# voxel-tracer/ag-pathtracer

Measured on AMD Instinct MI355X. Metric: Mrays/sec (primary+secondary) at 1080p/64spp, higher is better.
Workload: dtype f32; 1 GPU; BASELINE configs[2]: Sponza-class closed atrium, 258672 tris / 37 primitives / 35 Disney materials, 1920x1080, 64 spp, PathTracer MaxDepth=5, NEE+MIS; triangles=258672, spp=64

## Files before the change

### ag-pathtracer_amd/csrc/agpt_api.hip

```cpp
#include <hip/hip_runtime.h>

#include <algorithm>
#include <cstdlib>
#include <cstring>
#include <memory>
#include <string>
#include <vector>

#include "agpt_adaptive.h"
#include "agpt_denoise.h"
#include "agpt_internal.h"
#include "agpt_kernels.h"

namespace agpt {

static thread_local std::string g_error;

int fail(int code, const std::string& msg) {
    g_error = msg;
    return code;
}

int interleave_rows(int H, int block, int world, int rank) {
    int rows = 0;
    for (int k = rank, y = k * block; y < H; k += world, y = k * block) rows += std::min(block, H - y);
    return rows;
}

}
using agpt::fail;

static int trace_grid(const agpt_ctx* c) { return c->num_cus * c->blocks_per_cu; }
static int fast_grid(const agpt_ctx* c) { return c->num_cus * c->fast_blocks_per_cu; }

static bool use_fast_trace(const agpt_ctx* c, const DevScene& sc, int count) {
    return count != 1 && sc.n_prims <= 64 * AGPT_MAX_CHUNKS && !c->force_generic;
}

#define AGPT_SMALL_BATCH (48ull << 20)

struct TraceLaunch {
    hipStream_t stream;
    const uint32_t* queue;
    const uint32_t* count_ptr;
    uint32_t count_imm;
    uint32_t* work_head;
    float4 *ro, *rd;
    DevHit* hits;
    uint32_t* occ;
    int count;
    bool small_batch;
    bool recast;
};

template <int MODE, bool COUNT, bool SPILL, bool PEEK>
static void launch_trace_fast(agpt_ctx* c, const DevScene& sc, const TraceLaunch& t) {
    const dim3 block(AGPT_BLOCK), g(fast_grid(c));
    const int refill = MODE == 0 ? c->refill : c->refill_any;
    if (sc.n_prims <= 64) {
        hipLaunchKernelGGL((k_trace_fast<MODE, AGPT_FAST_STACK, false, COUNT, SPILL, PEEK>), g, block, 0, t.stream, sc, t.queue, t.count_ptr,
                           t.count_imm, t.work_head, t.ro, t.rd, t.hits, t.occ, c->counters.p,
                           refill, 0u, c->spill.p, (const unsigned long long*)nullptr, (const uint32_t*)nullptr, MODE == 0 && t.recast,
                           (const float4*)c->beta4.p, c->L4.p);
        return;
    }
    const uint32_t stride = (uint32_t)c->pool_paths;
    if (c->cand_chunks.n < c->pool_paths || c->cand_mask.n < (size_t)((sc.n_prims + 63) / 64) * c->pool_paths) {
        c->note(hipErrorOutOfMemory);
        return;
    }
    hipLaunchKernelGGL((k_candidates<MODE>), dim3(c->num_cus * 8), block, 0, t.stream, sc, t.queue, t.count_ptr, t.count_imm, t.ro, t.rd,
                       c->cand_mask.p, c->cand_chunks.p, stride);
    hipLaunchKernelGGL((k_trace_fast<MODE, AGPT_FAST_STACK, true, COUNT, SPILL, PEEK>), g, block, 0, t.stream, sc, t.queue, t.count_ptr,
                       t.count_imm, t.work_head, t.ro, t.rd, t.hits, t.occ, c->counters.p, refill, stride, c->spill.p,
                       (const unsigned long long*)c->cand_mask.p, (const uint32_t*)c->cand_chunks.p, false, (const float4*)nullptr,
                       (float4*)nullptr);
}

template <bool ANY, bool COUNT, int DEPTH>
static void launch_trace_generic(agpt_ctx* c, int grid, const DevScene& sc, const TraceLaunch& t) {
    hipLaunchKernelGGL((k_trace<ANY, COUNT, DEPTH>), dim3(grid), dim3(AGPT_BLOCK), 0, t.stream, sc, t.queue, t.count_ptr, t.count_imm,
                       t.work_head, t.ro, t.rd, t.hits, t.occ, c->counters.p);
}

template <int MODE>
static void launch_trace(agpt_ctx* c, const DevScene& sc, const TraceLaunch& t) {
    constexpr bool ANY = MODE == 1;
    if (use_fast_trace(c, sc, t.count)) {
        const bool spill = sc.max_depth > AGPT_FAST_STACK;
        if (spill) {
            const size_t need = (size_t)(sc.max_depth - AGPT_FAST_STACK) * (size_t)fast_grid(c) * AGPT_BLOCK;
// ... 159 lines not shown
    if ((rc = c->work.ensure(4096))) return rc;
    if ((rc = c->counters.ensure(1))) return rc;
    c->pool_paths = paths;
    return AGPT_OK;
}

static int fit_pool(agpt_ctx* c, const agpt_scene* s, size_t unit, uint64_t& count) {
    if (unit * (size_t)count > c->pool_paths) {
        size_t free_b = 0, total_b = 0;
        if (hipMemGetInfo(&free_b, &total_b) == hipSuccess) {
            const size_t per_path = AGPT_BYTES_PER_PATH + candidate_bytes_per_path(s->dev.n_prims);
            const size_t avail = free_b + c->pool_paths * per_path;
            const size_t fit = (size_t)((double)avail * 0.9) / per_path;
            while (count > 1 && unit * (size_t)count > fit) count = (count + 1) / 2;
        }
    }
    int rc = ensure_pool(c, unit * (size_t)count, s->dev.n_prims);
    while (rc == AGPT_ERR_NOMEM && count > 1) {
        release_pool(c);
        count = (count + 1) / 2;
        rc = ensure_pool(c, unit * (size_t)count, s->dev.n_prims);
    }
    return rc;
}

static bool shade_tables_fit_lds(const DevScene& d) {
    return agpt::shade_tables_fit_lds(d.n_prims, d.n_materials, d.n_lights) && !getenv("AGPT_SHADE_GLOBAL_TABLES");
}

struct WavefrontRun {
    PathBuffers pb;
    Queues q[2];
    bool mis_mode, timing;
    int count;
    agpt::ShadeVariant shade;
    uint64_t iterations = 0, launches = 0;
};

static int begin_wavefront(agpt_ctx* c, const agpt_scene* s, int enable_counters, bool timing, WavefrontRun& run) {
#define X(T, name) run.pb.name = c->name.p;
    AGPT_POOL_BUFFERS(X)
#undef X
    for (int i = 0; i < 2; i++) {
        Queues& q = run.q[i];
        q.ext = c->q[i][0].p; q.mis = c->q[i][1].p; q.shadow = c->q[i][2].p;
        q.counts = c->qcounts.p + AGPT_NQUEUES * AGPT_QSTRIDE * i;
    }
    run.count = enable_counters == 2 ? 2 : (enable_counters != 0 ? 1 : 0);
    run.mis_mode = use_fast_trace(c, s->dev, run.count) && !c->mis_closest;
    run.timing = timing;
    run.shade.fast = s->shading_arith == AGPT_SHADING_FAST;
    run.shade.level = s->shade_level;
    run.shade.lds_tables = shade_tables_fit_lds(s->dev);
    run.shade.env = !s->envs.empty();
    c->tev_used = 0;
    c->tev_kind.clear();
    HIP_TRY(hipMemsetAsync(c->counters.p, 0, sizeof(DevCounters), c->stream));
    HIP_TRY(hipEventRecord(c->ev[0], c->stream));
    return AGPT_OK;
}

static void set_wavefront_consts(RenderConsts& rc, const WavefrontRun& run, int max_depth, bool trace_all_rays) {
    rc.max_depth = max_depth;
    rc.mis_mode = run.mis_mode ? 1 : 0;
    rc.answer_rays = (run.mis_mode && !trace_all_rays) ? 1 : 0;
}

static int run_wavefront(agpt_ctx* c, agpt_scene* s, const RenderConsts& rcn, WavefrontRun& run) {
    const int count = run.count;
    const PathBuffers& pb = run.pb;
    Queues* const q = run.q;
    const int shade_grid = c->num_cus * c->shade_blocks_per_cu;
    const bool small_batch = (unsigned long long)rcn.NP * (unsigned long long)rcn.S < AGPT_SMALL_BATCH;
    const bool recast = !getenv("AGPT_NO_RECAST");
    const bool side = (c->multi_stream == 2 || (c->multi_stream == 1 && small_batch)) && use_fast_trace(c, s->dev, count) &&
                      s->dev.max_depth <= AGPT_FAST_STACK && s->dev.n_prims <= 64;
    const hipStream_t main_stream = c->stream, mis_stream = side ? c->aux_stream[0] : main_stream,
                      shadow_stream = side ? c->aux_stream[1] : main_stream;
    int cur = 0;
    const int planned = rcn.max_depth + 2;
    for (int it = 0;; it++) {
        if (it >= planned) {
            uint32_t* slot = c->host_pinned + (it & 1) * (AGPT_NQUEUES * AGPT_QSTRIDE);
            HIP_TRY(hipMemcpyAsync(slot, q[cur].counts, ((AGPT_NQUEUES - 1) * AGPT_QSTRIDE + 1) * sizeof(uint32_t), hipMemcpyDeviceToHost, main_stream));
            HIP_TRY(hipEventRecord(c->ev[2 + (it & 1)], main_stream));
            if (it > planned) {
                const uint32_t* seen = c->host_pinned + ((it - 1) & 1) * (AGPT_NQUEUES * AGPT_QSTRIDE);
                HIP_TRY(hipEventSynchronize(c->ev[2 + ((it - 1) & 1)]));
                if (seen[0] == 0 && seen[AGPT_QSTRIDE] == 0 && seen[2 * AGPT_QSTRIDE] == 0) break;
            }
            if (it > 4096) return fail(AGPT_ERR_LIMIT, "agpt: path did not terminate");
        }
        const int nxt = cur ^ 1;
        HIP_TRY(hipMemsetAsync(q[nxt].counts, 0, AGPT_NQUEUES * AGPT_QSTRIDE * sizeof(uint32_t), main_stream));
        HIP_TRY(hipMemsetAsync(c->work.p, 0, 4 * AGPT_FRONTIERS * AGPT_QSTRIDE * sizeof(uint32_t), main_stream));
        uint32_t* const heads[4] = {c->work.p, c->work.p + AGPT_FRONTIERS * AGPT_QSTRIDE, c->work.p + 2 * AGPT_FRONTIERS * AGPT_QSTRIDE,
                                    c->work.p + 3 * AGPT_FRONTIERS * AGPT_QSTRIDE};
        const TraceLaunch ext{main_stream, q[cur].ext, &QCOUNT(q[cur], 0), 0, heads[0], pb.ext_o, pb.ext_d, pb.hit, nullptr,
                              count, small_batch, recast};
        const TraceLaunch mis{mis_stream, q[cur].mis, &QCOUNT(q[cur], 1), 0, heads[1], pb.mis_o, pb.mis_d,
                              run.mis_mode ? nullptr : pb.mis_hit, run.mis_mode ? pb.mis_ok : nullptr, count, small_batch, false};
        const TraceLaunch shadow{shadow_stream, q[cur].shadow, &QCOUNT(q[cur], 2), 0, heads[2], pb.sh_o, pb.sh_d, nullptr, pb.occluded,
                                 count, small_batch, false};
        auto trace_ext = [&]() { launch_trace_timed<0>(c, run.timing, 0, s->dev, ext); };
        auto trace_mis = [&]() {
            if (run.mis_mode) launch_trace_timed<2>(c, run.timing, 1, s->dev, mis);
            else launch_trace_timed<0>(c, run.timing, 1, s->dev, mis);
        };
        auto trace_shadow = [&]() { launch_trace_timed<1>(c, run.timing, 2, s->dev, shadow); };
        if (side) {
            HIP_TRY(hipEventRecord(c->aux_ev[0], main_stream));
            HIP_TRY(hipStreamWaitEvent(mis_stream, c->aux_ev[0], 0));
            HIP_TRY(hipStreamWaitEvent(shadow_stream, c->aux_ev[0], 0));
            trace_mis();
            HIP_TRY(hipEventRecord(c->aux_ev[1], mis_stream));
            trace_shadow();
            HIP_TRY(hipEventRecord(c->aux_ev[2], shadow_stream));
            trace_ext();
            HIP_TRY(hipStreamWaitEvent(main_stream, c->aux_ev[1], 0));
            HIP_TRY(hipStreamWaitEvent(main_stream, c->aux_ev[2], 0));
        } else {
            trace_ext();
            trace_mis();
            trace_shadow();
        }
        agpt::launch_shading(main_stream, run.shade, shade_grid, s->dev, rcn, pb, q[cur], q[nxt], c->counters.p, heads[3]);
        cur = nxt;
        run.iterations++;
        run.launches += 3;
    }
    return AGPT_OK;
}

static void read_counters(const DevCounters& d, agpt_stats* st) {
    st->closest_rays = d.closest_rays;
    st->anyhit_rays = d.anyhit_rays;
// ... 1 lines not shown
    st->root_tests = d.roots;
    st->tri_tests = d.tris;
    st->shaded_vertices = d.shaded;
    st->outliers = d.outliers;
    st->samples = d.samples;
    st->answered_rays = d.answered;
}

static int end_wavefront(agpt_ctx* c) {
    HIP_TRY(hipEventRecord(c->ev[1], c->stream));
    HIP_TRY(hipGetLastError());
    HIP_TRY(c->take_deferred());
    return AGPT_OK;
}

static int fill_stats(agpt_ctx* c, const WavefrontRun& run, uint64_t samples, agpt_stats* stats) {
    if (!stats) return AGPT_OK;
    HIP_TRY(hipStreamSynchronize(c->stream));
    std::memset(stats, 0, sizeof(*stats));
    DevCounters dc;
    HIP_TRY(hipMemcpy(&dc, c->counters.p, sizeof(dc), hipMemcpyDeviceToHost));
    read_counters(dc, stats);
#ifdef AGPT_SHADE_CLOCK
    {
        const double tot = (double)dc.dbg[55];
        static const char* names[8] = {"record loads", "resolve pending", "surface", "emission/termination", "BSDF set-up + light sampling",
                                       "evaluations + ray stores", "final stores", "queue appends + barriers"};
        std::fprintf(stderr, "[shade clock] wave-cycles %.4g:", tot);
        for (int k = 0; k < 8; ++k) std::fprintf(stderr, "  %s %.1f%%", names[k], 100. * dc.dbg[56 + k] / tot);
        std::fprintf(stderr, "\n");
    }
#endif
#ifdef AGPT_TRACE_STATS
    for (int mode = 0; mode < 3; ++mode) {
        const unsigned long long* d = dc.dbg + 16 * mode;
        const double steps = (double)(d[0] + d[1] + d[2]);
        if (steps == 0) continue;
        std::fprintf(stderr,
                     "[trace stats mode %d] steps A/B/C %.3g/%.3g/%.3g (%.1f%%/%.1f%%/%.1f%%)  lanes per step A %.1f B %.1f C %.1f  "
                     "active lanes per step %.1f  refills %.3g (%.1f lanes each)  prefilter batches %.3g\n", mode,
                     (double)d[0], (double)d[1], (double)d[2], 100 * d[0] / steps, 100 * d[1] / steps, 100 * d[2] / steps,
                     d[0] ? (double)d[3] / d[0] : 0., d[1] ? (double)d[4] / d[1] : 0., d[2] ? (double)d[5] / d[2] : 0.,
                     (double)d[6] / steps, (double)d[7], d[7] ? (double)d[8] / d[7] : 0., (double)d[9]);
#ifndef AGPT_TRACE_CLOCK
        std::fprintf(stderr, "[trace stats mode %d] stack pushes %.3g: to depth > 4 %.2f%%  > 6 %.3f%%  > 8 %.4f%%  > 12 %.5f%%\n", mode, (double)d[10],
                     d[10] ? 100. * d[11] / d[10] : 0., d[10] ? 100. * d[12] / d[10] : 0., d[10] ? 100. * d[13] / d[10] : 0.,
                     d[10] ? 100. * d[14] / d[10] : 0.);
#endif
#ifdef AGPT_TRACE_CLOCK
        const double tot = (double)dc.dbg[48 + mode];
        std::fprintf(stderr,
                     "[trace clock mode %d] wave-cycles %.4g: refill %.1f%%  vote %.1f%%  B %.1f%% (of which load wait %.1f%%)  C %.1f%%  A %.1f%%;"
                     "  cycles per step: B %.0f (wait %.0f)  C %.0f  A %.0f  vote %.0f; per refill %.0f\n", mode, tot,
                     100 * d[10] / tot, 100 * d[11] / tot, 100 * d[13] / tot, 100 * d[12] / tot, 100 * d[14] / tot, 100 * d[15] / tot,
                     d[1] ? (double)d[13] / d[1] : 0., d[1] ? (double)d[12] / d[1] : 0., d[2] ? (double)d[14] / d[2] : 0.,
                     d[0] ? (double)d[15] / d[0] : 0., (double)d[11] / steps, d[7] ? (double)d[10] / d[7] : 0.);
#endif
    }
#endif
    stats->samples = samples;
    stats->iterations = run.iterations;
    stats->trace_launches = run.launches;
    float ms = 0;
    HIP_TRY(hipEventElapsedTime(&ms, c->ev[0], c->ev[1]));
    stats->total_ms = ms;
    if (run.timing) {
        for (size_t i = 0; i + 1 < c->tev_used; i += 2) {
            float t = 0;
            HIP_TRY(hipEventElapsedTime(&t, c->tev[i], c->tev[i + 1]));
            const int kind = c->tev_kind[i / 2];
// ... 11 lines not shown
    return AGPT_OK;
}
static int check_tile(const char* fn, const agpt_render_params* rp) {
    if (rp->width <= 0 || rp->height <= 0 || rp->w <= 0 || rp->h <= 0 || rp->x0 < 0 || rp->y0 < 0 || rp->x0 + rp->w > rp->width ||
        rp->y0 + rp->h > rp->height || rp->accum_pitch < rp->x0 + rp->w)
        return fail(AGPT_ERR_INVALID, std::string(fn) + ": bad tile / film");
    return AGPT_OK;
}

static int tile_rows(const char* fn, const agpt_render_params* rp, uint32_t& rows) {
    rows = (uint32_t)rp->h;
    if (rp->interleave_block <= 0) return AGPT_OK;
    if (rp->interleave_world < 1 || rp->interleave_rank < 0 || rp->interleave_rank >= rp->interleave_world || rp->x0 != 0 ||
        rp->y0 != 0 || rp->w != rp->width || rp->h != rp->height)
        return fail(AGPT_ERR_INVALID, std::string(fn) + ": row interleave needs the whole film as tile and 0 <= rank < world");
    rows = (uint32_t)agpt::interleave_rows(rp->height, rp->interleave_block, rp->interleave_world, rp->interleave_rank);
    return AGPT_OK;
}

static RenderConsts tile_consts(const agpt_render_params* rp, uint32_t NP) {
    RenderConsts rc{};
    rc.W = rp->width; rc.H = rp->height; rc.x0 = rp->x0; rc.y0 = rp->y0; rc.w = rp->w; rc.h = rp->h;
    rc.accum_pitch = rp->accum_pitch; rc.accum_row0 = rp->accum_row0; rc.NP = NP;
    rc.il_block = rp->interleave_block; rc.il_world = rp->interleave_world; rc.il_rank = rp->interleave_rank;
    return rc;
}

static uint64_t samples_per_batch(const agpt_render_params* rp, uint32_t NP) {
    return rp->samples_per_batch > 0 ? (uint64_t)rp->samples_per_batch : std::max<uint64_t>(1, (128ull << 20) / NP);
}

static void trace_rays(agpt_ctx* c, const DevScene& sc, uint32_t n, bool any_hit, int count) {
    const TraceLaunch t{c->stream, nullptr, nullptr, n, c->work.p, c->ext_o.p, c->ext_d.p, c->hit.p, c->occluded.p,
                        count, (unsigned long long)n < AGPT_SMALL_BATCH, false};
    if (any_hit) launch_trace<1>(c, sc, t);
    else launch_trace<0>(c, sc, t);
}

int agpt_intersect_device(agpt_scene* s, const agpt_ray* d_rays, int n, agpt_hit* d_out, int any_hit, agpt_stats* stats) {
    if (!s || !d_rays || !d_out || n < 0) return fail(AGPT_ERR_INVALID, "agpt_intersect_device: bad argument");
    if (!s->committed) return fail(AGPT_ERR_INVALID, "agpt_intersect_device: scene not committed");
    if (n == 0) return AGPT_OK;
    agpt_ctx* c = s->ctx;
    HIP_TRY(hipSetDevice(c->device));
    int rc = ensure_pool(c, (size_t)n, s->dev.n_prims);
    if (rc) return rc;
    HIP_TRY(hipMemsetAsync(c->counters.p, 0, sizeof(DevCounters), c->stream));
    HIP_TRY(hipMemsetAsync(c->work.p, 0, AGPT_FRONTIERS * AGPT_QSTRIDE * sizeof(uint32_t), c->stream));
    const dim3 blocks = agpt_blocks((uint64_t)n);
    hipLaunchKernelGGL(k_prepare_rays, blocks, dim3(AGPT_BLOCK), 0, c->stream, d_rays, n, c->ext_o.p, c->ext_d.p);
    HIP_TRY(hipEventRecord(c->ev[0], c->stream));
    const int instrumented = (stats != nullptr && !getenv("AGPT_INTERSECT_TIMING")) ? 1 : 0;
    trace_rays(c, s->dev, (uint32_t)n, any_hit != 0, instrumented);
    HIP_TRY(hipEventRecord(c->ev[1], c->stream));
    hipLaunchKernelGGL(k_export_hits, blocks, dim3(AGPT_BLOCK), 0, c->stream, s->dev, c->hit.p, c->occluded.p, n, any_hit,
                       d_out);
    HIP_TRY(hipStreamSynchronize(c->stream));
    HIP_TRY(hipGetLastError());
    HIP_TRY(c->take_deferred());
    WavefrontRun one{};
    one.launches = 1;
    if ((rc = fill_stats(c, one, 0, stats))) return rc;
    if (stats) stats->trace_ms = stats->total_ms;
    return AGPT_OK;
}

int agpt_intersect_batch(agpt_scene* s, const agpt_ray* rays, int n, agpt_hit* out, int any_hit, agpt_stats* stats) {
// ... 6 lines not shown
    DevBuf<agpt_hit> d_out;
    if (d_rays.alloc((size_t)n) != hipSuccess || d_out.alloc((size_t)n) != hipSuccess)
        return fail(AGPT_ERR_NOMEM, "agpt_intersect_batch: out of device memory");
    HIP_TRY(hipMemcpyAsync(d_rays.p, rays, (size_t)n * sizeof(agpt_ray), hipMemcpyHostToDevice, c->stream));
    int rc = agpt_intersect_device(s, d_rays.p, n, d_out.p, any_hit, stats);
    if (rc) return rc;
    HIP_TRY(hipMemcpy(out, d_out.p, (size_t)n * sizeof(agpt_hit), hipMemcpyDeviceToHost));
    return AGPT_OK;
}

int agpt_render(agpt_scene* s, const agpt_render_params* rp, float* accum_dev, agpt_stats* stats) {
    if (!s || !rp || !accum_dev) return fail(AGPT_ERR_INVALID, "agpt_render: NULL argument");
    if (!s->committed || !s->has_camera) return fail(AGPT_ERR_INVALID, "agpt_render: scene not committed or camera not set");
    int rc;
    if ((rc = check_tile("agpt_render", rp)) || (rc = check_depth("agpt_render", rp->max_depth))) return rc;
    if (rp->spp_count < 0) return fail(AGPT_ERR_INVALID, "agpt_render: bad sample range");
    agpt_ctx* c = s->ctx;
    HIP_TRY(hipSetDevice(c->device));
    uint32_t rows;
    if ((rc = tile_rows("agpt_render", rp, rows))) return rc;
    if (rows == 0) return AGPT_OK;
    const uint32_t NP = (uint32_t)rp->w * rows;
    uint64_t batch = std::min<uint64_t>(samples_per_batch(rp, NP), (uint64_t)std::max(1, rp->spp_count));
    if ((uint64_t)NP * batch > 0x7FFFFFFFull) return fail(AGPT_ERR_LIMIT, "agpt_render: batch too large");
    if ((rc = fit_pool(c, s, NP, batch))) return rc;
    const int S = (int)batch;
    s->dev.cam = s->cam;

    WavefrontRun run;
    if ((rc = begin_wavefront(c, s, rp->enable_counters, rp->enable_timing != 0 && stats != nullptr, run))) return rc;
    RenderConsts rcn = tile_consts(rp, NP);
    rcn.seed_base = rp->seed_base;
    set_wavefront_consts(rcn, run, rp->max_depth, rp->trace_all_rays != 0);
    for (int s0 = rp->spp_begin; s0 < rp->spp_begin + rp->spp_count; s0 += S) {
        rcn.s0 = s0;
        rcn.S = std::min(S, rp->spp_begin + rp->spp_count - s0);
        const uint32_t total = NP * (uint32_t)rcn.S;
        hipLaunchKernelGGL(k_generate, agpt_blocks(total), dim3(AGPT_BLOCK), 0, c->stream, s->dev, rcn, run.pb,
                           run.q[0]);
        if ((rc = run_wavefront(c, s, rcn, run))) return rc;
        agpt::launch_accumulate(c->stream, run.shade.fast, s->dev, rcn, run.pb, (float4*)accum_dev, c->counters.p);
    }
    if ((rc = end_wavefront(c))) return rc;
    return fill_stats(c, run, (uint64_t)NP * (uint64_t)rp->spp_count, stats);
}

int agpt_render_adaptive(agpt_scene* s, const agpt_render_params* rp, const agpt_adaptive_params* ap, float* accum_dev,
                         float* moment2_dev, agpt_stats* stats, agpt_adaptive_stats* astats) {
    if (!s || !rp || !ap || !accum_dev || !moment2_dev) return fail(AGPT_ERR_INVALID, "agpt_render_adaptive: NULL argument");
    if (!s->committed || !s->has_camera) return fail(AGPT_ERR_INVALID, "agpt_render_adaptive: scene not committed or camera not set");
    int rc;
    if ((rc = check_tile("agpt_render_adaptive", rp)) || (rc = check_depth("agpt_render_adaptive", rp->max_depth))) return rc;
    if (rp->spp_begin != 0 || rp->spp_count != 0)
        return fail(AGPT_ERR_INVALID, "agpt_render_adaptive: spp_begin and spp_count must be 0 (the counts are in accum.w)");
    const int step = ap->step_spp, min_spp = ap->min_spp, max_spp = ap->max_spp;
    if (step < 1 || min_spp < 2 || min_spp > max_spp || max_spp > (1 << 24) || min_spp % step != 0 || max_spp % step != 0 ||
        !(ap->abs_floor >= 0.f) || ap->rel_error != ap->rel_error)
        return fail(AGPT_ERR_INVALID, "agpt_render_adaptive: need 1 <= step_spp, 2 <= min_spp <= max_spp <= 2^24, both multiples of "
                                      "step_spp, abs_floor >= 0, rel_error not NaN");
    if (astats) std::memset(astats, 0, sizeof(*astats));
    agpt_ctx* c = s->ctx;
    HIP_TRY(hipSetDevice(c->device));
    uint32_t rows;
    if ((rc = tile_rows("agpt_render_adaptive", rp, rows))) return rc;
    if (rows == 0) return AGPT_OK;
    const uint32_t NP = (uint32_t)rp->w * rows;
// ... 156 lines not shown
```

### ag-pathtracer_amd/csrc/agpt_kernels.h

```cpp
#pragma once

#include <type_traits>

#include "agpt_shade.h"
#include "agpt_trace.h"

#include "agpt_wavefront.h"

template <bool ANY, bool COUNT, int DEPTH>
__global__ void __launch_bounds__(AGPT_BLOCK)
k_trace(DevScene sc, const uint32_t* __restrict__ queue, const uint32_t* __restrict__ count_ptr, uint32_t count_imm,
        uint32_t* __restrict__ work_head, const float4* __restrict__ ray_o, const float4* __restrict__ ray_d,
        DevHit* __restrict__ hits, uint32_t* __restrict__ occluded, DevCounters* __restrict__ counters) {
    __shared__ uint32_t s_stack[DEPTH * AGPT_BLOCK];
    uint32_t* stack = s_stack + threadIdx.x;
    const int lane = threadIdx.x & 63;
    const uint32_t count = count_ptr ? *count_ptr : count_imm;
    TraceCounters cnt;
    cnt.interior = 0;
    cnt.tris = 0;
    cnt.roots = 0;
    cnt.last_mesh = 0;
    for (;;) {
        uint32_t base = 0;
// ... 9 lines not shown
            if (ANY)
                occluded[pid] = hit ? 1u : 0u;
            else
                hits[pid] = h;
        }
    }
    if (COUNT) {
        for (int off = 32; off > 0; off >>= 1) {
            cnt.interior += __shfl_down(cnt.interior, off);
            cnt.tris += __shfl_down(cnt.tris, off);
            cnt.roots += __shfl_down(cnt.roots, off);
        }
        if (lane == 0) {
            atomicAdd(&counters->interior, (unsigned long long)cnt.interior);
            atomicAdd(&counters->tris, (unsigned long long)cnt.tris);
            atomicAdd(&counters->roots, (unsigned long long)cnt.roots);
        }
    }
    if (threadIdx.x == 0 && blockIdx.x == 0) {
        if (ANY)
            atomicAdd(&counters->anyhit_rays, (unsigned long long)count);
        else
            atomicAdd(&counters->closest_rays, (unsigned long long)count);
    }
}

#define AGPT_RING 128

#ifndef AGPT_TRACE_WAVES
#define AGPT_TRACE_WAVES 1
#endif
template <int MODE, bool LIST>
using TraceRays = std::conditional_t<MODE == 0 && !LIST, float4*, const float4* __restrict__>;
template <int MODE, int DEPTH, bool LIST, bool COUNT, bool SPILL, bool PEEK>
__global__ void __launch_bounds__(AGPT_BLOCK, AGPT_TRACE_WAVES)
k_trace_fast(DevScene sc, const uint32_t* __restrict__ queue, const uint32_t* __restrict__ count_ptr, uint32_t count_imm,
             uint32_t* __restrict__ work_head, TraceRays<MODE, LIST> ray_o, TraceRays<MODE, LIST> ray_d,
             DevHit* __restrict__ hits, uint32_t* __restrict__ occluded, DevCounters* __restrict__ counters, int refill,
             uint32_t cand_stride, uint32_t* __restrict__ spill, const unsigned long long* __restrict__ cand_mask,
             const uint32_t* __restrict__ cand_chunks, bool recast_on, const float4* path_beta4, float4* path_L4) {
    constexpr bool ANY = MODE != 0;
    constexpr bool MIS = MODE == 2;
    constexpr int BLOCK = AGPT_BLOCK;
    constexpr bool PRIM_LDS = !LIST;
    __shared__ uint32_t s_stack[DEPTH * BLOCK];
    __shared__ float4 s_prim[PRIM_LDS ? 2 * 64 : 2];
    uint32_t* stack = s_stack + threadIdx.x;
    uint32_t* spill_col = SPILL ? spill + (size_t)blockIdx.x * BLOCK + threadIdx.x : nullptr;
    const size_t spill_stride = (size_t)gridDim.x * BLOCK;
    auto stack_push = [&](int k, uint32_t v) {
        if (!SPILL || k < DEPTH)
            stack[k * BLOCK] = v;
        else
            spill_col[(size_t)(k - DEPTH) * spill_stride] = v;
    };
    auto stack_at = [&](int k) -> uint32_t {
        if (!SPILL || k < DEPTH) return stack[k * BLOCK];
        return spill_col[(size_t)(k - DEPTH) * spill_stride];
    };
    const int lane = threadIdx.x & 63;
    const unsigned long long lt_mask = (1ull << lane) - 1ull;
    const uint32_t count = (uint32_t)__builtin_amdgcn_readfirstlane((int)(count_ptr ? *count_ptr : count_imm));
    if (blockIdx.x * (uint32_t)BLOCK >= count) return;
    const int n_prims = LIST ? 0 : sc.n_prims;
    if (PRIM_LDS && (int)threadIdx.x < n_prims) {
        const DevPrim& P = sc.prims[threadIdx.x];
        float4 a, b;
        if (P.type == AGPT_PRIM_SPHERE) {
            a.x = P.cx; a.y = P.cy; a.z = P.cz; a.w = 1.f;
            b.x = P.r2; b.y = 0.f; b.z = P.material < 0 ? 1.f : 0.f; b.w = 0.f;
        } else if (P.type == AGPT_PRIM_PLANE) {
            a.x = P.cx; a.y = P.cy; a.z = P.cz; a.w = 3.f;
            b.x = P.r; b.y = P.r2; b.z = P.material < 0 ? 1.f : 0.f; b.w = 0.f;
        } else {
            a.x = P.root_bmin[0]; a.y = P.root_bmin[1]; a.z = P.root_bmin[2]; a.w = P.n_tris > 0 ? 0.f : 2.f;
            b.x = P.root_bmax[0]; b.y = P.root_bmax[1]; b.z = P.root_bmax[2]; b.w = __uint_as_float(P.root_enc);
// ... 39 lines not shown
            return rootpair_base + 2u * (uint32_t)(__ffsll((long long)low) - 1);
        }
        return CUR_PICK;
    };
    auto enter_chunk = [&](uint32_t c) {
        cvisit &= ~(1u << c);
        cchunk = c;
        mask = cand_mask[(size_t)c * cand_stride + pid];
        mmask = sc.chunk_mesh_masks[c];
    };
    uint32_t seg = blockIdx.x & (AGPT_FRONTIERS - 1u), segs_left = AGPT_FRONTIERS;
    const uint32_t seg_len = ((count + AGPT_FRONTIERS - 1u) / AGPT_FRONTIERS + 63u) & ~63u;
    uint32_t cur = CUR_IDLE, hid = AGPT_HIT_MISS;
    int sp = 0;
    float rayt = 0.f, hb1 = 0.f, hb2 = 0.f;
    TraceRay r;
    r.O = V3s(0.f);
    r.D = V3(0.f, 0.f, 1.f);
    r.R = V3s(1.f);
    r.fast = true;

    __shared__ uint32_t s_ring_pid[BLOCK / 64][AGPT_RING];
    __shared__ unsigned long long s_ring_mask[BLOCK / 64][AGPT_RING];
    uint32_t* ring_pid = s_ring_pid[threadIdx.x >> 6];
    unsigned long long* ring_mask = s_ring_mask[threadIdx.x >> 6];
    uint32_t ring_head = 0, ring_tail = 0;
    bool mis_area = false;
    int mis_skip = -1;
    bool mis_reach = true;
    bool any_slow = false;
    uint32_t c_int = 0, c_root = 0, c_tri = 0;
    TS(unsigned long long ts_steps[3] = {0, 0, 0}; unsigned long long ts_lanes[3] = {0, 0, 0}; unsigned long long ts_act = 0;
       unsigned long long ts_refills = 0; unsigned long long ts_refilled = 0; unsigned long long ts_pref = 0;
       uint32_t ts_push[5] = {0, 0, 0, 0, 0};)
    TCK(unsigned long long tk_refill = 0, tk_vote = 0, tk_bmem = 0, tk_balu = 0, tk_c = 0, tk_a = 0; const unsigned long long tk_begin = TCK_NOW();)

    uint32_t pfa_off = 0;
    uint32_t pfa_seg = 0;
    bool pfa_valid = false;
    uint32_t pfb_pid = 0, pfb_n = 0;
    bool pfb_valid = false;
    uint32_t pfc_pid = 0, pfc_n = 0;
    bool pfc_valid = false;
    float4 pfc_o, pfc_d;
    pfc_o.x = 0.f; pfc_o.y = 0.f; pfc_o.z = 0.f; pfc_o.w = 0.f;
    pfc_d = pfc_o;
    auto drained = [&]() -> bool { return segs_left == 0 && !pfa_valid && !pfb_valid && !pfc_valid; };
    auto pin_state = [&]() {
        seg = uni(seg); segs_left = uni(segs_left); ring_tail = uni(ring_tail); ring_head = uni(ring_head);
        pfa_seg = uni(pfa_seg); pfa_valid = uni(pfa_valid); pfb_n = uni(pfb_n); pfb_valid = uni(pfb_valid);
        pfc_n = uni(pfc_n); pfc_valid = uni(pfc_valid);
    };
    auto pump_consume = [&]() {
        if (LIST) {
            if (pfc_valid) {
                if ((uint32_t)lane < pfc_n) {
                    const uint32_t slot = (ring_tail + (uint32_t)lane) & (AGPT_RING - 1);
                    ring_pid[slot] = pfc_pid;
                    ring_mask[slot] = (unsigned long long)__float_as_uint(pfc_o.x);
                }
                ring_tail += pfc_n;
                pfc_valid = false;
                TS(ts_pref++;)
            }
        } else if (pfc_valid) {
            if ((uint32_t)lane < pfc_n) {
                const uint32_t npid = pfc_pid;
// ... 185 lines not shown
                            mis_area = true;
                            mis_skip = (int)shape;
                            mis_reach = sphere_test_c(lc, lr2, r, rayt, ts);
                            if (mis_reach) rayt = ts;
                        }
                    }
                    hid = AGPT_HIT_MISS;
                    hb1 = 0.f;
                    hb2 = 0.f;
                    sp = 0;
                    cur = pick_next(mask);
                }
            }
            ring_head += take;
            TS(ts_refills++; ts_refilled += take;)
            if (!pfc_valid && !drained()) pump_issue();
            act = __ballot(cur != CUR_IDLE);
            any_slow = __ballot(cur != CUR_IDLE && !r.fast) != 0;
        }
        TCK(tk_refill += TCK_NOW() - tk_r0;)
        if (act == 0) break;

        for (;;) {
            TCK(const unsigned long long tk_v0 = TCK_NOW();)
            const int nA = __popcll(__ballot(LIST ? cur - CUR_FETCH < 2u : cur == CUR_PICK)), nB = __popcll(__ballot(cur < CUR_B_END)),
                      nC = __popcll(__ballot((int32_t)cur < 0));
            const int n_active = nA + nB + nC;
            if (n_active == 0 || (n_active <= 64 - refill && !(drained() && ring_head == ring_tail))) break;
            if (MODE == 0 && !LIST && n_active <= 64 - refill && __ballot(cur == CUR_RECAST) != 0) break;
            TCK(const unsigned long long tk_v1 = TCK_NOW(); tk_vote += tk_v1 - tk_v0;)
            TS(ts_act += (unsigned long long)n_active; if (!(nB >= nA && nB >= nC) && !(nC >= nA)) { ts_steps[0]++; ts_lanes[0] += nA; })
            if (nB >= nA && nB >= nC) {
                TS(ts_steps[1]++; ts_lanes[1] += nB;)
                if (cur < CUR_B_END) {
                    if (MODE != 1) __builtin_amdgcn_s_setprio(1);
                    const NodePair np = load_pair(sc, cur);
                    if (MODE != 1) {
                        asm volatile("" ::: "memory");
                        __builtin_amdgcn_s_setprio(0);
                    }
                    TCK(asm volatile("s_waitcnt vmcnt(0)" ::: "memory"); tk_bmem += TCK_NOW() - tk_v1;)
                    float dl, dr;
                    bool hl, hr;
                    const uint32_t encl = __float_as_uint(np.n3.x), encr = __float_as_uint(np.n3.y);
                    pair_boxes_fast(np, r, rayt, hl, hr, dl, dr);
                    if (any_slow) {
                        if (!r.fast) pair_boxes_exact(np, r, rayt, hl, hr, dl, dr);
                    }
                    if (COUNT) {
                        if (cur < rootpair_base) c_int++; else c_root++;
                    }
                    hr = hr && cur < rootpair_base;
                    if (hl && hr) {
                        bool swap = ANY ? false : (dr < dl);
                        stack_push(sp, swap ? encl : encr);
                        sp++;
                        TS(ts_push[0]++; ts_push[1] += sp > 4; ts_push[2] += sp > 6; ts_push[3] += sp > 8; ts_push[4] += sp > 12;)
                        cur = swap ? encr : encl;
                    } else if (hl) {
                        cur = encl;
                    } else if (hr) {
                        cur = encr;
                    } else if (sp == 0) {
                        cur = pick_next(mask);
                    } else {
                        sp--;
                        cur = stack_at(sp);
                    }
                }
                TCK(asm volatile("s_waitcnt lgkmcnt(0)" ::: "memory"); tk_balu += TCK_NOW() - tk_v1;)
            } else if (nC >= nA) {
                TS(ts_steps[2]++; ts_lanes[2] += nC;)
                if ((int32_t)cur < 0) {
                    uint32_t first, cnt;
                    leaf_range(sc, cur, first, cnt);
                    bool done = false;
                    for (uint32_t i = 0; i < cnt; ++i) {
                        const float4* tp = sc.tri_verts + 3 * (size_t)(first + i);
                        const float4 a = tp[0], b = tp[1], c = tp[2];
                        const v3 q0 = V3(a.x, a.y, a.z), q1 = V3(b.x, b.y, b.z), q2 = V3(c.x, c.y, c.z);
                        const uint32_t q_id = __float_as_uint(a.w), q_flags = __float_as_uint(b.w);
                        float t, b1, b2;
                        if (COUNT) c_tri++;
                        if (tri_test(q0, q1, q2, r, rayt, t, b1, b2)) {
                            if (MIS) {
                                if (!(q_flags & AGPT_TRI_FLAG_REJECT)) {
                                    done = true;
                                    break;
                                }
                            } else if (ANY) {
                                done = true;
                                break;
                            } else if (!(q_flags & AGPT_TRI_FLAG_REJECT)) {
                                rayt = t;
                                hid = q_id;
                                hb1 = b1;
                                hb2 = b2;
                            }
                        }
                    }
                    if (ANY && done) {
                        occluded[pid] = MIS ? 0u : 1u;
                        cur = CUR_IDLE;
                    } else if (sp == 0) {
                        cur = pick_next(mask);
                    } else {
// ... 28 lines not shown
                        const bool sphere = P.type == AGPT_PRIM_SPHERE;
                        pa.x = P.cx; pa.y = P.cy; pa.z = P.cz; pa.w = sphere ? 1.f : (P.type == AGPT_PRIM_PLANE ? 3.f : 2.f);
                        pb2.x = sphere ? P.r2 : P.r; pb2.y = sphere ? 0.f : P.r2; pb2.z = 0.f; pb2.w = 0.f;
                    } else {
                        pa = s_prim[2 * k];
                        pb2 = s_prim[2 * k + 1];
                    }
                    if (pa.w == 1.f || pa.w == 3.f) {
                        float root;
                        if (analytic_test(pa.w, V3(pa.x, pa.y, pa.z), pb2.x, pb2.y, r, rayt, root)) {
                            if (MIS) {
                                const bool tie_loses = pa.w == 1.f && mis_area && mis_reach && k < mis_skip && root == rayt;
                                if (!tie_loses) {
                                    occluded[pid] = 0u;
                                    cur = CUR_IDLE;
                                }
                            } else if (ANY) {
                                occluded[pid] = 1u;
                                cur = CUR_IDLE;
                            } else {
                                rayt = root;
                                hid = AGPT_HIT_SPHERE | (uint32_t)k;
                                hb1 = 0.f;
                                hb2 = 0.f;
                            }
                        }
                    }
                    if (cur == CUR_PICK) cur = pick_next(mask);
                }
                TCK(asm volatile("s_waitcnt lgkmcnt(0)" ::: "memory"); tk_a += TCK_NOW() - tk_v1;)
            }
        }
    }
    TS(if (lane == 0) {
        unsigned long long* d = counters->dbg + 16 * MODE;
        for (int k = 0; k < 3; ++k) { atomicAdd(d + k, ts_steps[k]); atomicAdd(d + 3 + k, ts_lanes[k]); }
        atomicAdd(d + 6, ts_act); atomicAdd(d + 7, ts_refills); atomicAdd(d + 8, ts_refilled); atomicAdd(d + 9, ts_pref);
    })
#if defined(AGPT_TRACE_STATS) && !defined(AGPT_TRACE_CLOCK)
    {
        unsigned long long* d = counters->dbg + 16 * MODE;
        for (int k = 0; k < 5; ++k) {
            uint32_t v = ts_push[k];
            for (int off = 32; off > 0; off >>= 1) v += __shfl_down(v, off);
            if (lane == 0) atomicAdd(d + 10 + k, (unsigned long long)v);
        }
    }
#endif
    TS(if (lane == 0) {
        unsigned long long* d = counters->dbg + 16 * MODE;
        TCK(atomicAdd(d + 10, tk_refill); atomicAdd(d + 11, tk_vote); atomicAdd(d + 12, tk_bmem); atomicAdd(d + 13, tk_balu);
            atomicAdd(d + 14, tk_c); atomicAdd(d + 15, tk_a); atomicAdd(counters->dbg + 48 + MODE, TCK_NOW() - tk_begin);)
    })
    if (COUNT) {
        for (int off = 32; off > 0; off >>= 1) {
            c_int += __shfl_down(c_int, off);
            c_root += __shfl_down(c_root, off);
            c_tri += __shfl_down(c_tri, off);
        }
        if (lane == 0) {
            atomicAdd(&counters->interior, (unsigned long long)c_int);
            atomicAdd(&counters->roots, (unsigned long long)c_root);
            atomicAdd(&counters->tris, (unsigned long long)c_tri);
        }
    }
    if (threadIdx.x == 0 && blockIdx.x == 0) {
        if (MODE == 1)
            atomicAdd(&counters->anyhit_rays, (unsigned long long)count);
        else
            atomicAdd(&counters->closest_rays, (unsigned long long)count);
    }
}

static_assert(AGPT_MAX_CHUNKS <= 32, "k_trace_fast<LIST> and k_candidates keep the chunks still to visit in one 32-bit word per ray");
#define AGPT_CAND_LIST 24
template <int MODE>
__global__ void __launch_bounds__(AGPT_BLOCK)
k_candidates(DevScene sc, const uint32_t* __restrict__ queue, const uint32_t* __restrict__ count_ptr, uint32_t count_imm,
             const float4* __restrict__ ray_o, const float4* __restrict__ ray_d, unsigned long long* __restrict__ cand_mask,
             uint32_t* __restrict__ cand_chunks, uint32_t cand_stride) {
    constexpr bool MIS = MODE == 2;
    __shared__ uint16_t s_list[AGPT_CAND_LIST][AGPT_BLOCK];
    const uint32_t count = count_ptr ? *count_ptr : count_imm;
    const int n_chunks = (sc.n_prims + 63) / 64;
    const int tid = threadIdx.x;
// ... 140 lines not shown
```

### ag-pathtracer_amd/csrc/agpt_wavefront.h

```cpp
#pragma once

#include "agpt_math.h"
#include "agpt_scene.h"

#define AGPT_BLOCK 256
#define AGPT_CHUNK 64

#define PF_BOUNCE_MASK 0xFFu
#define PF_SPECULAR 0x100u
#define PF_DEAD 0x200u
#define PF_PEND_C1 0x400u
#define PF_PEND_C2 0x800u
#define PF_PENDING 0x1000u

struct PathBuffers {
    float4 *ext_o, *ext_d;
    float4 *sh_o, *sh_d;
    float4 *mis_o, *mis_d;
    DevHit *hit, *mis_hit;
    uint32_t* occluded;
    uint32_t* mis_ok;
    float4* beta4;
    float4* L4;
    float4* fac4;
// ... 84 lines not shown
    b4.x = 1.f; b4.y = 1.f; b4.z = 1.f; b4.w = __uint_as_float(0u);
    l4.x = 0.f; l4.y = 0.f; l4.z = 0.f; l4.w = __uint_as_float(rng);
    pb.ext_o[i] = o4;
    pb.ext_d[i] = d4;
    pb.beta4[i] = b4;
    pb.L4[i] = l4;
    q.ext[i] = i;
    if (i == 0) {
        QCOUNT(q, 0) = total;
        QCOUNT(q, 1) = 0;
        QCOUNT(q, 2) = 0;
    }
}
struct FilmSample { v3 clr; uint32_t bad; };
__device__ __forceinline__ FilmSample film_sample(v3 clr, uint32_t bad) {
    if (isnan(clr.x) || isnan(clr.y) || isnan(clr.z) || isinf(luminance(clr))) {
        clr = V3s(0.f);
        bad++;
    }
    return FilmSample{clr, bad};
}
__device__ __forceinline__ uint32_t resolve_word(const float4& a, float n) {
    float e = 1 / 2.2f;
    float r = powf(a.x / n, e), g = powf(a.y / n, e), b = powf(a.z / n, e);
    int ri = (int)(256 * tclampf(r, 0.0f, 0.999f));
    int gi = (int)(256 * tclampf(g, 0.0f, 0.999f));
    int bi = (int)(256 * tclampf(b, 0.0f, 0.999f));
    return (uint32_t)((ri << 16) + (gi << 8) + bi);
}

struct DevCounters {
    unsigned long long closest_rays, anyhit_rays, interior, tris, shaded, outliers, samples, roots, answered;
#if defined(AGPT_TRACE_STATS) || defined(AGPT_SHADE_CLOCK)
    unsigned long long dbg[64];
#endif
};
#ifdef AGPT_TRACE_STATS
#define TS(...) __VA_ARGS__
#else
#define TS(...)
#endif
#ifdef AGPT_TRACE_CLOCK
#define TCK(...) __VA_ARGS__
#define TCK_NOW() __builtin_amdgcn_s_memtime()
#else
#define TCK(...)
#endif

__device__ __forceinline__ uint32_t uni(uint32_t v) { return (uint32_t)__builtin_amdgcn_readfirstlane((int)v); }
__device__ __forceinline__ bool uni(bool v) { return __builtin_amdgcn_readfirstlane((int)v) != 0; }

__device__ __forceinline__ void queue_push(uint32_t* q, uint32_t* count, bool pred, uint32_t value) {
    unsigned long long mask = __ballot(pred);
    if (mask == 0) return;
    int lane = __lane_id();
    int leader = __ffsll((long long)mask) - 1;
    uint32_t base = 0;
    if (lane == leader) base = atomicAdd(count, (uint32_t)__popcll(mask));
    base = __shfl(base, leader);
    if (pred) {
        uint32_t off = (uint32_t)__popcll(mask & ((1ull << lane) - 1ull));
        q[base + off] = value;
    }
}


namespace agpt {
// ... 19 lines not shown
```

Before: 4205 Mrays/s.

## Add coherent primary-ray trace variant using scalar loads for wave-uniform nodes and leaves

Adds a COH instantiation of the fast trace kernel. It is used only for the first extension bounce of camera rays when samples are grouped 64 per pixel and the scene has at most 64 primitives. When every active lane in a wave visits the same BVH node or leaf, the node pair and triangle data are read once through scalar constant-address-space loads instead of per-lane vector loads. The variant also fixes refill at 64 and uses a different launch-bounds occupancy hint. It adds a per-step ballot and readlane check that costs extra work when lanes diverge, and it doubles code paths in the traversal loop.

```diff
diff --git a/ag-pathtracer_amd/csrc/agpt_api.hip b/ag-pathtracer_amd/csrc/agpt_api.hip
--- a/ag-pathtracer_amd/csrc/agpt_api.hip
+++ b/ag-pathtracer_amd/csrc/agpt_api.hip
@@ -51,12 +51,21 @@
     int count;
     bool small_batch;
     bool recast;
+    bool coherent;
 };
 
 template <int MODE, bool COUNT, bool SPILL, bool PEEK>
 static void launch_trace_fast(agpt_ctx* c, const DevScene& sc, const TraceLaunch& t) {
     const dim3 block(AGPT_BLOCK), g(fast_grid(c));
     const int refill = MODE == 0 ? c->refill : c->refill_any;
+    if constexpr (MODE == 0 && !COUNT) {
+        if (t.coherent && sc.n_prims <= 64) {
+            hipLaunchKernelGGL((k_trace_fast<0, AGPT_FAST_STACK, false, false, SPILL, PEEK, true>), g, block, 0, t.stream, sc, t.queue,
+                               t.count_ptr, t.count_imm, t.work_head, t.ro, t.rd, t.hits, t.occ, c->counters.p, 64, 0u, c->spill.p,
+                               (const unsigned long long*)nullptr, (const uint32_t*)nullptr, t.recast, (const float4*)c->beta4.p, c->L4.p);
+            return;
+        }
+    }
     if (sc.n_prims <= 64) {
         hipLaunchKernelGGL((k_trace_fast<MODE, AGPT_FAST_STACK, false, COUNT, SPILL, PEEK>), g, block, 0, t.stream, sc, t.queue, t.count_ptr,
                            t.count_imm, t.work_head, t.ro, t.rd, t.hits, t.occ, c->counters.p,
@@ -282,6 +291,7 @@
     PathBuffers pb;
     Queues q[2];
     bool mis_mode, timing;
+    bool camera_rays = false;
     int count;
     agpt::ShadeVariant shade;
     uint64_t iterations = 0, launches = 0;
@@ -323,6 +333,8 @@
     const int shade_grid = c->num_cus * c->shade_blocks_per_cu;
     const bool small_batch = (unsigned long long)rcn.NP * (unsigned long long)rcn.S < AGPT_SMALL_BATCH;
     const bool recast = !getenv("AGPT_NO_RECAST");
+    const bool coherent = run.camera_rays && sample_group(rcn.S) == 64 && use_fast_trace(c, s->dev, count) && s->dev.n_prims <= 64 &&
+                          count == 0 && !getenv("AGPT_NO_COHERENT");
     const bool side = (c->multi_stream == 2 || (c->multi_stream == 1 && small_batch)) && use_fast_trace(c, s->dev, count) &&
                       s->dev.max_depth <= AGPT_FAST_STACK && s->dev.n_prims <= 64;
     const hipStream_t main_stream = c->stream, mis_stream = side ? c->aux_stream[0] : main_stream,
@@ -347,11 +359,11 @@
         uint32_t* const heads[4] = {c->work.p, c->work.p + AGPT_FRONTIERS * AGPT_QSTRIDE, c->work.p + 2 * AGPT_FRONTIERS * AGPT_QSTRIDE,
                                     c->work.p + 3 * AGPT_FRONTIERS * AGPT_QSTRIDE};
         const TraceLaunch ext{main_stream, q[cur].ext, &QCOUNT(q[cur], 0), 0, heads[0], pb.ext_o, pb.ext_d, pb.hit, nullptr,
-                              count, small_batch, recast};
+                              count, small_batch, recast, coherent && it == 0};
         const TraceLaunch mis{mis_stream, q[cur].mis, &QCOUNT(q[cur], 1), 0, heads[1], pb.mis_o, pb.mis_d,
-                              run.mis_mode ? nullptr : pb.mis_hit, run.mis_mode ? pb.mis_ok : nullptr, count, small_batch, false};
+                              run.mis_mode ? nullptr : pb.mis_hit, run.mis_mode ? pb.mis_ok : nullptr, count, small_batch, false, false};
         const TraceLaunch shadow{shadow_stream, q[cur].shadow, &QCOUNT(q[cur], 2), 0, heads[2], pb.sh_o, pb.sh_d, nullptr, pb.occluded,
-                                 count, small_batch, false};
+                                 count, small_batch, false, false};
         auto trace_ext = [&]() { launch_trace_timed<0>(c, run.timing, 0, s->dev, ext); };
         auto trace_mis = [&]() {
             if (run.mis_mode) launch_trace_timed<2>(c, run.timing, 1, s->dev, mis);
@@ -419,10 +431,15 @@
     }
 #endif
 #ifdef AGPT_TRACE_STATS
-    for (int mode = 0; mode < 3; ++mode) {
-        const unsigned long long* d = dc.dbg + 16 * mode;
+    for (int mode = 0; mode < 4; ++mode) {
+        const unsigned long long* d = dc.dbg + (mode < 3 ? 16 * mode : AGPT_DBG_COH);
         const double steps = (double)(d[0] + d[1] + d[2]);
         if (steps == 0) continue;
+        if (mode == 3)
+            std::fprintf(stderr, "[trace stats mode 3] scalar path: B %.3g of %.3g wave-steps (%.1f%%), %.3g of %.3g lane-steps (%.1f%%);  "
+                         "C %.3g of %.3g wave-steps (%.1f%%), %.3g of %.3g lane-steps (%.1f%%)\n",
+                         (double)d[16], (double)d[1], d[1] ? 100. * d[16] / d[1] : 0., (double)d[18], (double)d[4], d[4] ? 100. * d[18] / d[4] : 0.,
+                         (double)d[17], (double)d[2], d[2] ? 100. * d[17] / d[2] : 0., (double)d[19], (double)d[5], d[5] ? 100. * d[19] / d[5] : 0.);
         std::fprintf(stderr,
                      "[trace stats mode %d] steps A/B/C %.3g/%.3g/%.3g (%.1f%%/%.1f%%/%.1f%%)  lanes per step A %.1f B %.1f C %.1f  "
                      "active lanes per step %.1f  refills %.3g (%.1f lanes each)  prefilter batches %.3g\n", mode,
@@ -500,7 +517,7 @@
 
 static void trace_rays(agpt_ctx* c, const DevScene& sc, uint32_t n, bool any_hit, int count) {
     const TraceLaunch t{c->stream, nullptr, nullptr, n, c->work.p, c->ext_o.p, c->ext_d.p, c->hit.p, c->occluded.p,
-                        count, (unsigned long long)n < AGPT_SMALL_BATCH, false};
+                        count, (unsigned long long)n < AGPT_SMALL_BATCH, false, false};
     if (any_hit) launch_trace<1>(c, sc, t);
     else launch_trace<0>(c, sc, t);
 }
@@ -573,6 +590,7 @@
     RenderConsts rcn = tile_consts(rp, NP);
     rcn.seed_base = rp->seed_base;
     set_wavefront_consts(rcn, run, rp->max_depth, rp->trace_all_rays != 0);
+    run.camera_rays = true;
     for (int s0 = rp->spp_begin; s0 < rp->spp_begin + rp->spp_count; s0 += S) {
         rcn.s0 = s0;
         rcn.S = std::min(S, rp->spp_begin + rp->spp_count - s0);
diff --git a/ag-pathtracer_amd/csrc/agpt_kernels.h b/ag-pathtracer_amd/csrc/agpt_kernels.h
--- a/ag-pathtracer_amd/csrc/agpt_kernels.h
+++ b/ag-pathtracer_amd/csrc/agpt_kernels.h
@@ -65,8 +65,8 @@
 #endif
 template <int MODE, bool LIST>
 using TraceRays = std::conditional_t<MODE == 0 && !LIST, float4*, const float4* __restrict__>;
-template <int MODE, int DEPTH, bool LIST, bool COUNT, bool SPILL, bool PEEK>
-__global__ void __launch_bounds__(AGPT_BLOCK, AGPT_TRACE_WAVES)
+template <int MODE, int DEPTH, bool LIST, bool COUNT, bool SPILL, bool PEEK, bool COH = false>
+__global__ void __launch_bounds__(AGPT_BLOCK, COH ? 5 : AGPT_TRACE_WAVES)
 k_trace_fast(DevScene sc, const uint32_t* __restrict__ queue, const uint32_t* __restrict__ count_ptr, uint32_t count_imm,
              uint32_t* __restrict__ work_head, TraceRays<MODE, LIST> ray_o, TraceRays<MODE, LIST> ray_d,
              DevHit* __restrict__ hits, uint32_t* __restrict__ occluded, DevCounters* __restrict__ counters, int refill,
@@ -74,7 +74,9 @@
              const uint32_t* __restrict__ cand_chunks, bool recast_on, const float4* path_beta4, float4* path_L4) {
     constexpr bool ANY = MODE != 0;
     constexpr bool MIS = MODE == 2;
+    static_assert(!COH || (MODE == 0 && !LIST && !COUNT), "the coherent instantiation is a plain short-list closest-hit launch");
     constexpr int BLOCK = AGPT_BLOCK;
+    if constexpr (COH) refill = 64;
     constexpr bool PRIM_LDS = !LIST;
     __shared__ uint32_t s_stack[DEPTH * BLOCK];
     __shared__ float4 s_prim[PRIM_LDS ? 2 * 64 : 2];
@@ -180,7 +182,8 @@
     uint32_t c_int = 0, c_root = 0, c_tri = 0;
     TS(unsigned long long ts_steps[3] = {0, 0, 0}; unsigned long long ts_lanes[3] = {0, 0, 0}; unsigned long long ts_act = 0;
        unsigned long long ts_refills = 0; unsigned long long ts_refilled = 0; unsigned long long ts_pref = 0;
-       uint32_t ts_push[5] = {0, 0, 0, 0, 0};)
+       uint32_t ts_push[5] = {0, 0, 0, 0, 0};
+       unsigned long long ts_usteps[2] = {0, 0}; unsigned long long ts_ulanes[2] = {0, 0};)
     TCK(unsigned long long tk_refill = 0, tk_vote = 0, tk_bmem = 0, tk_balu = 0, tk_c = 0, tk_a = 0; const unsigned long long tk_begin = TCK_NOW();)
 
     uint32_t pfa_off = 0;
@@ -432,7 +435,55 @@
             TS(ts_act += (unsigned long long)n_active; if (!(nB >= nA && nB >= nC) && !(nC >= nA)) { ts_steps[0]++; ts_lanes[0] += nA; })
             if (nB >= nA && nB >= nC) {
                 TS(ts_steps[1]++; ts_lanes[1] += nB;)
-                if (cur < CUR_B_END) {
+                if constexpr (COH) {
+                    auto interior = [&](const NodePair& np) {
+                        float dl, dr;
+                        bool hl, hr;
+                        const uint32_t encl = __float_as_uint(np.n3.x), encr = __float_as_uint(np.n3.y);
+                        pair_boxes_fast(np, r, rayt, hl, hr, dl, dr);
+                        if (any_slow) {
+                            if (!r.fast) pair_boxes_exact(np, r, rayt, hl, hr, dl, dr);
+                        }
+                        hr = hr && cur < rootpair_base;
+                        if (hl && hr) {
+                            const bool swap = dr < dl;
+                            stack_push(sp, swap ? encl : encr);
+                            sp++;
+                            TS(ts_push[0]++; ts_push[1] += sp > 4; ts_push[2] += sp > 6; ts_push[3] += sp > 8; ts_push[4] += sp > 12;)
+                            cur = swap ? encr : encl;
+                        } else if (hl) {
+                            cur = encl;
+                        } else if (hr) {
+                            cur = encr;
+                        } else if (sp == 0) {
+                            cur = pick_next(mask);
+                        } else {
+                            sp--;
+                            cur = stack_at(sp);
+                        }
+                    };
+                    const bool in_b = cur < CUR_B_END;
+                    const uint32_t u = (uint32_t)__builtin_amdgcn_readlane((int)cur, __ffsll((long long)__ballot(in_b)) - 1);
+                    if (__ballot(in_b && cur != u) == 0) {
+                        TS(ts_usteps[0]++; ts_ulanes[0] += nB;)
+                        typedef const float __attribute__((address_space(4))) ConstF;
+                        ConstF* q = (ConstF*)sc.nodes + 8 * (size_t)u;
+                        NodePair np;
+                        np.n0.x = q[0]; np.n0.y = q[1]; np.n0.z = q[2]; np.n0.w = q[3];
+                        np.n1.x = q[4]; np.n1.y = q[5]; np.n1.z = q[6]; np.n1.w = q[7];
+                        np.n2.x = q[8]; np.n2.y = q[9]; np.n2.z = q[10]; np.n2.w = q[11];
+                        np.n3.x = q[12]; np.n3.y = q[13]; np.n3.z = q[14]; np.n3.w = q[15];
+                        asm volatile("" : "+s"(np.n0.x), "+s"(np.n0.y), "+s"(np.n0.z), "+s"(np.n0.w), "+s"(np.n1.x), "+s"(np.n1.y), "+s"(np.n1.z),
+                                     "+s"(np.n1.w), "+s"(np.n2.x), "+s"(np.n2.y), "+s"(np.n2.z), "+s"(np.n2.w), "+s"(np.n3.x), "+s"(np.n3.y));
+                        if (in_b) interior(np);
+                    } else if (in_b) {
+                        __builtin_amdgcn_s_setprio(1);
+                        const NodePair np = load_pair(sc, cur);
+                        asm volatile("" ::: "memory");
+                        __builtin_amdgcn_s_setprio(0);
+                        interior(np);
+                    }
+                } else if (cur < CUR_B_END) {
                     if (MODE != 1) __builtin_amdgcn_s_setprio(1);
                     const NodePair np = load_pair(sc, cur);
                     if (MODE != 1) {
@@ -471,7 +522,49 @@
                 TCK(asm volatile("s_waitcnt lgkmcnt(0)" ::: "memory"); tk_balu += TCK_NOW() - tk_v1;)
             } else if (nC >= nA) {
                 TS(ts_steps[2]++; ts_lanes[2] += nC;)
-                if ((int32_t)cur < 0) {
+                const bool in_c = (int32_t)cur < 0;
+                bool same_leaf = false;
+                uint32_t u = 0;
+                if constexpr (COH) {
+                    u = (uint32_t)__builtin_amdgcn_readlane((int)cur, __ffsll((long long)__ballot(in_c)) - 1);
+                    same_leaf = __ballot(in_c && cur != u) == 0;
+                }
+                if (COH && same_leaf) {
+                    TS(ts_usteps[1]++; ts_ulanes[1] += nC;)
+                    typedef const float __attribute__((address_space(4))) ConstF;
+                    typedef const uint32_t __attribute__((address_space(4))) ConstU;
+                    uint32_t first, cnt;
+                    if ((u & AGPT_ENC_BIGLEAF) == AGPT_ENC_BIGLEAF) {
+                        ConstU* bl = (ConstU*)sc.bigleaves + 2 * (size_t)(u & 0x0FFFFFFFu);
+                        first = bl[0];
+                        cnt = bl[1];
+                    } else {
+                        first = u & 0x0FFFFFFFu;
+                        cnt = ((u >> 28) & 7u) + 1u;
+                    }
+                    if (in_c) {
+                        for (uint32_t i = 0; i < cnt; ++i) {
+                            ConstF* tp = (ConstF*)sc.tri_verts + 12 * (size_t)(first + i);
+                            const v3 q0 = V3(tp[0], tp[1], tp[2]), q1 = V3(tp[4], tp[5], tp[6]), q2 = V3(tp[8], tp[9], tp[10]);
+                            const uint32_t q_id = __float_as_uint(tp[3]), q_flags = __float_as_uint(tp[7]);
+                            float t, b1, b2;
+                            if (tri_test(q0, q1, q2, r, rayt, t, b1, b2)) {
+                                if (!(q_flags & AGPT_TRI_FLAG_REJECT)) {
+                                    rayt = t;
+                                    hid = q_id;
+                                    hb1 = b1;
+                                    hb2 = b2;
+                                }
+                            }
+                        }
+                        if (sp == 0) {
+                            cur = pick_next(mask);
+                        } else {
+                            sp--;
+                            cur = stack_at(sp);
+                        }
+                    }
+                } else if ((int32_t)cur < 0) {
                     uint32_t first, cnt;
                     leaf_range(sc, cur, first, cnt);
                     bool done = false;
@@ -566,14 +659,16 @@
             }
         }
     }
+    TS(constexpr int TS_BASE = COH ? AGPT_DBG_COH : 16 * MODE;)
     TS(if (lane == 0) {
-        unsigned long long* d = counters->dbg + 16 * MODE;
+        unsigned long long* d = counters->dbg + TS_BASE;
+        if (COH) for (int k = 0; k < 2; ++k) { atomicAdd(d + 16 + k, ts_usteps[k]); atomicAdd(d + 18 + k, ts_ulanes[k]); }
         for (int k = 0; k < 3; ++k) { atomicAdd(d + k, ts_steps[k]); atomicAdd(d + 3 + k, ts_lanes[k]); }
         atomicAdd(d + 6, ts_act); atomicAdd(d + 7, ts_refills); atomicAdd(d + 8, ts_refilled); atomicAdd(d + 9, ts_pref);
     })
 #if defined(AGPT_TRACE_STATS) && !defined(AGPT_TRACE_CLOCK)
     {
-        unsigned long long* d = counters->dbg + 16 * MODE;
+        unsigned long long* d = counters->dbg + TS_BASE;
         for (int k = 0; k < 5; ++k) {
             uint32_t v = ts_push[k];
             for (int off = 32; off > 0; off >>= 1) v += __shfl_down(v, off);
@@ -582,9 +677,9 @@
     }
 #endif
     TS(if (lane == 0) {
-        unsigned long long* d = counters->dbg + 16 * MODE;
+        unsigned long long* d = counters->dbg + TS_BASE;
         TCK(atomicAdd(d + 10, tk_refill); atomicAdd(d + 11, tk_vote); atomicAdd(d + 12, tk_bmem); atomicAdd(d + 13, tk_balu);
-            atomicAdd(d + 14, tk_c); atomicAdd(d + 15, tk_a); atomicAdd(counters->dbg + 48 + MODE, TCK_NOW() - tk_begin);)
+            atomicAdd(d + 14, tk_c); atomicAdd(d + 15, tk_a); atomicAdd(counters->dbg + 48 + (COH ? 3 : MODE), TCK_NOW() - tk_begin);)
     })
     if (COUNT) {
         for (int off = 32; off > 0; off >>= 1) {
diff --git a/ag-pathtracer_amd/csrc/agpt_wavefront.h b/ag-pathtracer_amd/csrc/agpt_wavefront.h
--- a/ag-pathtracer_amd/csrc/agpt_wavefront.h
+++ b/ag-pathtracer_amd/csrc/agpt_wavefront.h
@@ -140,7 +140,8 @@
 struct DevCounters {
     unsigned long long closest_rays, anyhit_rays, interior, tris, shaded, outliers, samples, roots, answered;
 #if defined(AGPT_TRACE_STATS) || defined(AGPT_SHADE_CLOCK)
-    unsigned long long dbg[64];
+    unsigned long long dbg[96];
+#define AGPT_DBG_COH 64
 #endif
 };
 #ifdef AGPT_TRACE_STATS
```

Result: faster. 4251 Mrays/s (median of 6 runs) (+1.1%).
